# VisionDepth/VisionDepth3D

Measured on AMD Instinct MI355X. Metric: stereo-pairs/sec end-to-end (depth+warp+fill+mux), higher is better.
Workload: dtype f32; 1 GPU; 4k-dav2b-dibr; frame=3840x2160, format=Half-SBS, depth_model=depth-anything-v2-base, depth_net_dtype=float32 (the reference's precision), pixel_overlap=True, pixel_streams=2, clip_frames_all_ranks=32, params=render_cli.py defaults + dof_strength 2.0, dense DOF order (parity mode)

## Files before the change

include/vd3d.h:

```cpp
#ifndef VD3D_H
#define VD3D_H

#include <stddef.h>
#include <stdint.h>

#ifdef __cplusplus
extern "C" {
#endif

#define VD3D_ABI_VERSION 6

typedef enum vd3d_status {
  VD3D_OK = 0,
  VD3D_E_INVALID = -1,
  VD3D_E_HIP = -2,
  VD3D_E_NOMEM = -3,
  VD3D_E_UNSUPPORTED = -4
} vd3d_status;

typedef enum vd3d_format {
  VD3D_FMT_HALF_SBS = 0,
  VD3D_FMT_FULL_SBS = 1,
  VD3D_FMT_VR = 2,
  VD3D_FMT_ANAGLYPH = 3,
// ... 158 lines not shown
                         uint8_t* out_bgr, long long pitch_bytes);
int vd3d_add_weighted_u8(vd3d_ctx* ctx, const uint8_t* a, double alpha, const uint8_t* b, double beta, double gamma, long long n,
                         uint8_t* out);
int vd3d_rife_preprocess(vd3d_ctx* ctx, int dtype, const uint8_t* frame1_bgr, const uint8_t* frame2_bgr, int h, int w, int channels_last,
                         void* out6);
int vd3d_rife_postprocess(vd3d_ctx* ctx, const float* pred3, int h, int w, int channels_last, uint8_t* out_bgr);

int vd3d_conv3x3_c64_f16(vd3d_ctx* ctx, const void* x_nhwc, int H, int W, const void* w_frag, const float* bias, const float* slope_or_null,
                         void* y_nhwc);
int vd3d_conv3x3_head_f16(vd3d_ctx* ctx, const void* x_nhwc3, int H, int W, const float* w27x64, const float* bias, const float* slope_or_null,
                          void* y_nhwc64);
int vd3d_esr_tail_f32(vd3d_ctx* ctx, const void* t_nhwc64, const void* x_nhwc3, int H, int W, int r, float* out_planar);

int vd3d_depth_handoff(vd3d_ctx* ctx, const float* pred, int B, int ph, int pw, int H, int W, int invert, uint8_t* out_gray);

typedef enum vd3d_dtype { VD3D_DT_BF16 = 0, VD3D_DT_F32 = 1, VD3D_DT_F16 = 2  } vd3d_dtype;

int vd3d_depth_preprocess(vd3d_ctx* ctx, const uint8_t* frames_bgr, int B, int H, int W, int th, int tw,
                          const float* mean3_host, const float* std3_host, int dtype, void* out_nhwc);

int vd3d_add_layernorm(vd3d_ctx* ctx, int dtype, const void* x, const void* y_or_null, const void* gamma, const void* beta,
                       float eps, int64_t rows, int cols, void* out_sum, void* out_norm);

enum { VD3D_GEMM_EPI_NONE = 0, VD3D_GEMM_EPI_GELU = 1 };
enum { VD3D_X3_BF16X3 = 0, VD3D_X3_FP16X2 = 1 };
int64_t vd3d_gemm_x3_weight_bytes(int N, int K, int mode);
int vd3d_gemm_x3_pack_weights(vd3d_ctx* ctx, const float* W, int N, int K, int mode, void* image);
int vd3d_gemm_x3(vd3d_ctx* ctx, const float* X, int64_t M, int K, const void* w_image, int N, int mode, const float* bias_or_null, int epilogue, float* Y);
int64_t vd3d_attention_x3_workspace_bytes(int B, int T, int H, int D, int mode);
int vd3d_attention_x3(vd3d_ctx* ctx, const float* qkv, int B, int T, int H, int D, float scale, int mode, void* workspace, int64_t workspace_bytes, float* out);
int vd3d_attention_f32(vd3d_ctx* ctx, const float* qkv, int B, int T, int H, int D, float scale, float* out);

int64_t vd3d_conv3x3_x2_weight_bytes(int Cin, int Cout);
int vd3d_conv3x3_x2_pack_weights(vd3d_ctx* ctx, const float* W, int Cin, int Cout, void* image);
int vd3d_conv3x3_x2(vd3d_ctx* ctx, const float* X, int B, int H, int W, int Cin, const void* w_image, int Cout, float* Y);

int vd3d_upsample_bilinear_nhwc(vd3d_ctx* ctx, int dtype, const void* in, void* out, int B, int ih, int iw, int oh, int ow, int C);

int vd3d_nhwc_bias_act_f32(vd3d_ctx* ctx, const float* y, const float* bias_or_null, const float* r1_or_null, const float* r2_or_null, int relu,
                           int64_t n_pix, int C, float* out, float* relu_out_or_null);
int vd3d_upsample_bilinear_bias_nhwc_f32(vd3d_ctx* ctx, const float* in, const float* bias, float* out, int B, int ih, int iw, int oh, int ow, int C);
int vd3d_dpt_head_tail_f32(vd3d_ctx* ctx, const float* y, const float* b2, const float* w3, float b3, float scale, int64_t n_pix, int C, float* out);

int vd3d_depth_to_space_bias_nhwc_f32(vd3d_ctx* ctx, const float* y, const float* bias_or_null, int B, int H, int W, int s, int C, float* out);

typedef enum vd3d_preview {
  VD3D_PREVIEW_INTERLACED = 0,
  VD3D_PREVIEW_HSBS = 1,
  VD3D_PREVIEW_LR_DIFF = 2,
  VD3D_PREVIEW_FEATHER_BLEND = 3,
  VD3D_PREVIEW_RED_BLUE = 4
} vd3d_preview;
int vd3d_preview_image(vd3d_ctx* ctx, int type, const uint8_t* left_bgr, const uint8_t* right_bgr, int h, int w, uint8_t* out_bgr);
int vd3d_preview_heatmap(vd3d_ctx* ctx, int type, const float* shift_map, int h, int w, const uint8_t* lut_bgr_dev, uint8_t* out_bgr);
// ... 25 lines not shown
```

visiondepth3d_amd/_lib.py:

```python
from __future__ import annotations

import ctypes as C
import os

from . import _abi
from ._abi import FrameScalars, RenderParams, ShiftParams, State

_HERE = os.path.dirname(os.path.abspath(__file__))
LIB_PATH = os.environ.get("VD3D_LIB_PATH") or os.path.join(_HERE, "libvd3d_hip.so")

EXPORTS = (
    "vd3d_abi_version", "vd3d_last_error", "vd3d_shift_params_default", "vd3d_render_params_default",
    "vd3d_ctx_create", "vd3d_ctx_destroy", "vd3d_sync", "vd3d_ctx_stream", "vd3d_ctx_set_stream", "vd3d_ctx_pixel_stream", "vd3d_ctx_pixel_stream_k",
    "vd3d_state_reset", "vd3d_state_new_clip", "vd3d_state_export", "vd3d_state_import", "vd3d_state_planes",
    "vd3d_last_scalars", "vd3d_pixel_shift", "vd3d_render_frame", "vd3d_render_frame_blank", "vd3d_depth_handoff", "vd3d_heal_missing_pixels", "vd3d_preview_heatmap", "vd3d_preview_arrows", "vd3d_conv3x3_c64_f16", "vd3d_conv3x3_head_f16", "vd3d_esr_tail_f32", "vd3d_nv12_to_bgr", "vd3d_bgr_to_nv12", "vd3d_resize_cubic_u8", "vd3d_resize_area_u8", "vd3d_resize_linear_u8", "vd3d_format_3d_output", "vd3d_esr_preprocess", "vd3d_esr_postprocess", "vd3d_add_weighted_u8", "vd3d_rife_preprocess", "vd3d_rife_postprocess",
    "vd3d_shard_begin", "vd3d_shard_pixels", "vd3d_shard_pixels_blank", "vd3d_tdf_plane_export", "vd3d_tdf_plane_import", "vd3d_set_pixel_overlap", "vd3d_join_pixels", "vd3d_wait_pixels", "vd3d_finish_frame", "vd3d_quantiles",
    "vd3d_subject_depth", "vd3d_shard2_p0", "vd3d_shard2_set_crops", "vd3d_shard2_p1", "vd3d_shard2_p1_batch", "vd3d_shard2_r1", "vd3d_shard2_p3", "vd3d_shard2_p3_batch", "vd3d_shard2_r2", "vd3d_depth_preprocess", "vd3d_add_layernorm", "vd3d_gemm_x3_weight_bytes", "vd3d_gemm_x3_pack_weights", "vd3d_gemm_x3", "vd3d_attention_x3_workspace_bytes", "vd3d_attention_x3", "vd3d_attention_f32", "vd3d_conv3x3_x2_weight_bytes", "vd3d_conv3x3_x2_pack_weights", "vd3d_conv3x3_x2", "vd3d_upsample_bilinear_nhwc", "vd3d_nhwc_bias_act_f32", "vd3d_upsample_bilinear_bias_nhwc_f32", "vd3d_dpt_head_tail_f32", "vd3d_depth_to_space_bias_nhwc_f32", "vd3d_preview_image", "vd3d_detect_black_bars", "vd3d_stream_copy", "vd3d_torch_math", "vd3d_torch_math_aten", "vd3d_debug_gaussian_kernel1d", "vd3d_debug_exp_torch", "vd3d_set_profiling", "vd3d_last_stage_ms", "vd3d_stage_calls",
    "vd3d_debug_planes", "vd3d_debug_tune",
)

_lib = None


class Vd3dError(RuntimeError):
    def __init__(self, code, msg):
        super().__init__(f"libvd3d_hip error {code}: {msg}")
        self.code = code


def lib():
    global _lib
    if _lib is not None:
        return _lib
    if not os.path.exists(LIB_PATH):
        raise ImportError(f"{LIB_PATH} not built: run `python -c 'import __graft_entry__ as g; g.build()'` "
                          "(hipcc --offload-arch=gfx950). There is no CPU fallback.")
    L = C.CDLL(LIB_PATH)
    vp, i32, f32p, u8p = C.c_void_p, C.c_int, C.c_void_p, C.c_void_p
    L.vd3d_abi_version.restype = i32
    L.vd3d_last_error.restype = C.c_char_p
# ... 42 lines not shown
    L.vd3d_rife_preprocess.argtypes = [vp, i32, u8p, u8p, i32, i32, i32, vp]
    L.vd3d_rife_postprocess.argtypes = [vp, f32p, i32, i32, i32, u8p]
    L.vd3d_add_weighted_u8.argtypes = [vp, u8p, C.c_double, u8p, C.c_double, C.c_double, C.c_longlong, u8p]
    L.vd3d_finish_frame.argtypes = [vp, u8p, u8p, f32p, i32, i32, C.POINTER(RenderParams), C.c_double, i32, i32, u8p]
    L.vd3d_quantiles.argtypes = [vp, f32p, C.c_int64, C.POINTER(C.c_float), i32, C.POINTER(C.c_float)]
    L.vd3d_subject_depth.argtypes = [vp, f32p, i32, i32, C.POINTER(C.c_float)]
    L.vd3d_shard2_p0.argtypes = [vp, vp, vp, vp]
    L.vd3d_shard2_set_crops.argtypes = [vp, vp, i32]
    L.vd3d_shard2_p1.argtypes = [vp, vp, vp, i32, vp, i32, i32, vp]
    L.vd3d_shard2_p1_batch.argtypes = [vp, vp, vp, i32, vp, i32, i32, i32, vp]
    L.vd3d_shard2_p3_batch.argtypes = [vp, i32, i32, i32, vp, vp]
    L.vd3d_shard2_r1.argtypes = [vp, vp, i32]
    L.vd3d_shard2_p3.argtypes = [vp, i32, i32, vp, vp]
    L.vd3d_shard2_r2.argtypes = [vp, vp, C.POINTER(C.c_int), C.POINTER(C.c_uint8), i32, vp]
    L.vd3d_depth_preprocess.argtypes = [vp, vp, i32, i32, i32, i32, i32, C.POINTER(C.c_float), C.POINTER(C.c_float), i32, vp]
    L.vd3d_gemm_x3_weight_bytes.argtypes = [i32, i32, i32]
    L.vd3d_gemm_x3_weight_bytes.restype = C.c_int64
    L.vd3d_gemm_x3_pack_weights.argtypes = [vp, vp, i32, i32, i32, vp]
    L.vd3d_gemm_x3.argtypes = [vp, vp, C.c_int64, i32, vp, i32, i32, vp, i32, vp]
    L.vd3d_attention_x3_workspace_bytes.argtypes = [i32, i32, i32, i32, i32]
    L.vd3d_attention_x3_workspace_bytes.restype = C.c_int64
    L.vd3d_attention_x3.argtypes = [vp, vp, i32, i32, i32, i32, C.c_float, i32, vp, C.c_int64, vp]
    L.vd3d_attention_f32.argtypes = [vp, vp, i32, i32, i32, i32, C.c_float, vp]
    L.vd3d_conv3x3_x2_weight_bytes.argtypes = [i32, i32]
    L.vd3d_conv3x3_x2_weight_bytes.restype = C.c_int64
    L.vd3d_conv3x3_x2_pack_weights.argtypes = [vp, vp, i32, i32, vp]
    L.vd3d_conv3x3_x2.argtypes = [vp, vp, i32, i32, i32, i32, vp, i32, vp]
    L.vd3d_add_layernorm.argtypes = [vp, i32, vp, vp, vp, vp, C.c_float, C.c_int64, i32, vp, vp]
    L.vd3d_upsample_bilinear_nhwc.argtypes = [vp, i32, vp, vp, i32, i32, i32, i32, i32, i32]
    L.vd3d_nhwc_bias_act_f32.argtypes = [vp, vp, vp, vp, vp, i32, C.c_int64, i32, vp, vp]
    L.vd3d_upsample_bilinear_bias_nhwc_f32.argtypes = [vp, vp, vp, vp, i32, i32, i32, i32, i32, i32]
    L.vd3d_dpt_head_tail_f32.argtypes = [vp, vp, vp, vp, C.c_float, C.c_float, C.c_int64, i32, vp]
    L.vd3d_depth_to_space_bias_nhwc_f32.argtypes = [vp, vp, vp, i32, i32, i32, i32, i32, vp]
    L.vd3d_preview_image.argtypes = [vp, i32, vp, vp, i32, i32, vp]
    L.vd3d_detect_black_bars.argtypes = [vp, vp, i32, i32, C.POINTER(C.c_int), C.POINTER(C.c_int)]
    L.vd3d_stream_copy.argtypes = [vp, vp, vp, C.c_size_t]
    L.vd3d_torch_math.argtypes = [vp, i32, vp, C.c_float, vp, C.c_longlong]
    L.vd3d_torch_math_aten.argtypes = [vp, i32, vp, C.c_double, vp, C.c_longlong, i32]
    L.vd3d_debug_gaussian_kernel1d.argtypes = [i32, C.c_float, vp]
    L.vd3d_debug_exp_torch.argtypes = [vp, vp, C.c_longlong]
    L.vd3d_debug_tune.argtypes = [i32, i32]
    L.vd3d_set_profiling.argtypes = [vp, i32]
    L.vd3d_last_stage_ms.argtypes = [vp, C.c_char_p]
    L.vd3d_last_stage_ms.restype = C.c_float
    L.vd3d_stage_calls.argtypes = [vp, C.c_char_p]
    L.vd3d_stage_calls.restype = C.c_long
# ... 20 lines not shown
```

visiondepth3d_amd/csrc/vd3d_api.hip:

```cpp
#include <hip/hip_runtime.h>

#include <cmath>
#include <cstdarg>
#include <cstddef>
#include <cstdio>
#include <cstring>
#include <cstdlib>
#include <map>
#include <string>
#include <vector>

#include "vd3d_kernels.h"

#define VD3D_EXPORT extern "C" __attribute__((visibility("default")))

static thread_local char g_err[512] = "";
static int set_err(int code, const char* fmt, ...) {
  va_list ap;
  va_start(ap, fmt);
  vsnprintf(g_err, sizeof g_err, fmt, ap);
  va_end(ap);
  return code;
}
#define HIPCHK(x)                                                                                     \
// ... 1337 lines not shown
    return set_err(VD3D_E_UNSUPPORTED, "attention_f32: head size %d not built (64), an empty shape (B %d T %d H %d), B * H > 65535 or qkv / out not 16-byte aligned", D, B, T, H);
  HIPCHK(hipGetLastError());
  return 0;
}

VD3D_EXPORT int64_t vd3d_gemm_x3_weight_bytes(int N, int K, int mode) { return (int64_t)vd_gemm_x3_weight_bytes(N, K, mode); }

VD3D_EXPORT int vd3d_gemm_x3_pack_weights(vd3d_ctx* c, const float* W, int N, int K, int mode, void* image) {
  if (!c || !W || !image) return set_err(VD3D_E_INVALID, "bad argument");
  if (!vd_launch_gemm_x3_pack_w(c->stream, W, N, K, image, mode)) return set_err(VD3D_E_UNSUPPORTED, "gemm_x3: K %d must be a positive multiple of 16 (N %d), mode %d in {0, 1}", K, N, mode);
  HIPCHK(hipGetLastError());
  return 0;
}

VD3D_EXPORT int vd3d_gemm_x3(vd3d_ctx* c, const float* X, int64_t M, int K, const void* w_image, int N, int mode, const float* bias_or_null, int epilogue, float* Y) {
  if (!c || !X || !w_image || !Y || M < 1) return set_err(VD3D_E_INVALID, "bad argument");
  if (epilogue != VD3D_GEMM_EPI_NONE && epilogue != VD3D_GEMM_EPI_GELU) return set_err(VD3D_E_INVALID, "gemm_x3: unknown epilogue %d", epilogue);
  if (!vd_launch_gemm_x3(c->stream, X, (long long)M, K, w_image, N, bias_or_null, epilogue, Y, mode))
    return set_err(VD3D_E_UNSUPPORTED, "gemm_x3: K %d must be a positive multiple of 16, mode %d in {0, 1}, X and the weight image 16-byte aligned", K, mode);
  HIPCHK(hipGetLastError());
  return 0;
}

VD3D_EXPORT int vd3d_upsample_bilinear_nhwc(vd3d_ctx* c, int dtype, const void* in, void* out, int B, int ih, int iw, int oh, int ow, int C) {
  if (dtype != VD3D_DT_BF16 && dtype != VD3D_DT_F32) return set_err(VD3D_E_INVALID, "bad dtype %d", dtype);
  if (!c || !in || !out || B < 1 || ih < 1 || iw < 1) return set_err(VD3D_E_INVALID, "bad argument");
  if (!vd_launch_upsample_bilinear_nhwc(c->stream, dtype, in, out, B, ih, iw, oh, ow, C))
    return set_err(VD3D_E_UNSUPPORTED, "upsample_bilinear_nhwc: C not a multiple of 8 (bf16) / 4 (f32) or output smaller than 2x2");
  HIPCHK(hipGetLastError());
  return 0;
}

VD3D_EXPORT int vd3d_nhwc_bias_act_f32(vd3d_ctx* c, const float* y, const float* bias_or_null, const float* r1_or_null, const float* r2_or_null, int relu,
                                       int64_t n_pix, int C, float* out, float* relu_out_or_null) {
  if (!c || !y || !out || n_pix < 1 || C < 4) return set_err(VD3D_E_INVALID, "bad argument");
  HIPCHK(hipSetDevice(c->device));
  if (!vd_launch_bias_act_f32(c->stream, y, bias_or_null, r1_or_null, r2_or_null, relu, (long long)n_pix, C, out, relu_out_or_null))
    return set_err(VD3D_E_UNSUPPORTED, "nhwc_bias_act: C %d not a multiple of 4", C);
  HIPCHK(hipGetLastError());
  return 0;
}
VD3D_EXPORT int vd3d_upsample_bilinear_bias_nhwc_f32(vd3d_ctx* c, const float* in, const float* bias, float* out, int B, int ih, int iw, int oh, int ow, int C) {
  if (!c || !in || !bias || !out || B < 1 || ih < 1 || iw < 1) return set_err(VD3D_E_INVALID, "bad argument");
  HIPCHK(hipSetDevice(c->device));
  if (!vd_launch_upsample_bilinear_bias_nhwc_f32(c->stream, in, bias, out, B, ih, iw, oh, ow, C))
    return set_err(VD3D_E_UNSUPPORTED, "upsample_bilinear_bias_nhwc: C not a multiple of 4 or output smaller than 2x2");
// ... 183 lines not shown
```

visiondepth3d_amd/csrc/vd3d_gemm.hip:

```cpp
#include "vd3d_dev.h"
#include "vd3d_kernels.h"
#include <cstdlib>

typedef short gx_bf8 __attribute__((ext_vector_type(8)));
typedef float gx_f16 __attribute__((ext_vector_type(16)));

#define GX_BM 256
#define GX_BN 256
#define GX_NT 512
#define GX_MG 4
#define GX_A_STAGE (4 * GX_BM * 16)
#define GX_NTERM(MODE) ((MODE) == 0 ? 3 : 2)
#define GX_STAGE_HALF(MODE) (GX_NTERM(MODE) * 2 * GX_BN * 16)
#define GX_STAGE(MODE) (GX_A_STAGE + GX_STAGE_HALF(MODE))
#define GX_NSTAGE 4
#define GX_LDS(MODE) (GX_NSTAGE * GX_STAGE(MODE))

struct vd_gx_args {
  long long M;
  int K, N, KS;
  int nbm, nbn;
  int epilogue;
  int has_bias;
};

// ... 270 lines not shown
#endif
    attr_set = true;
  }
  vd_gx_args a;
  a.M = M; a.K = K; a.N = N; a.KS = K / 16;
  a.nbm = (int)((M + GX_BM - 1) / GX_BM); a.nbn = (N + GX_BN - 1) / GX_BN;
  a.epilogue = epilogue; a.has_bias = bias ? 1 : 0;
  const int per_xcd = (a.nbm + 7) / 8, groups = (per_xcd + GX_MG - 1) / GX_MG;
  const unsigned grid = 8u * (unsigned)groups * (unsigned)GX_MG * (unsigned)a.nbn;
  const float* cs = gx_colscale(wimg, N, K, mode);
  if (mode == 1) {
    hipLaunchKernelGGL((k_gemm_bf16x3<0, 1>), dim3(grid), dim3(GX_NT), GX_LDS(1), s, X, reinterpret_cast<const uint4*>(wimg), bias, cs, Y, a);
    return true;
  }
#ifdef VD_GEMM_ABLATE
#define GX_L(D) hipLaunchKernelGGL((k_gemm_bf16x3<D, 0>), dim3(grid), dim3(GX_NT), GX_LDS(0), s, X, reinterpret_cast<const uint4*>(wimg), bias, cs, Y, a)
  switch (dbg) { case 1: GX_L(1); return true; case 2: GX_L(2); return true; case 4: GX_L(4); return true; case 8: GX_L(8); return true; case 5: GX_L(5); return true;
                 case 3: GX_L(3); return true; case 9: GX_L(9); return true; case 11: GX_L(11); return true; case 16: GX_L(16); return true; case 27: GX_L(27); return true; case 32: GX_L(32); return true; case 64: GX_L(64); return true; case 128: GX_L(128); return true; case 130: GX_L(130); return true; case 256: GX_L(256); return true; default: break; }
#endif
  (void)dbg;
  hipLaunchKernelGGL((k_gemm_bf16x3<0, 0>), dim3(grid), dim3(GX_NT), GX_LDS(0), s, X, reinterpret_cast<const uint4*>(wimg), bias, cs, Y, a);
  return true;
}
```

visiondepth3d_amd/csrc/vd3d_kernels.h:

```cpp
#pragma once
#include <hip/hip_runtime.h>

#include "vd3d_work.h"

enum { VD_ST_A0 = 0, VD_ST_B0, VD_ST_A1, VD_ST_B1, VD_ST_A2, VD_ST_B2,
       VD_ST_AQ, VD_ST_BQ, VD_ST_BS };
#define PL_KMAX_HOST 129
#define DF_RMAX_HOST 15

#define VD_ETAB 8
struct vd_stage_args {
  int stage;
  int have_eye;
  int W, H;
  long long n_eye;
  long long n_crop;
  double ipd_factor;
  int shard;
  int shard_idx;
  float* q_out;
  long long* m_out;
  const int* crop_tab;
  const float* etab;
  int dbg;
// ... 137 lines not shown
                               int bar_width, int bar_side, uint8_t* L_out, uint8_t* R_out, const float* wtab);
#define VD_D4_WTAB_FLOATS (4 * 31 * 32)
bool vd_launch_sharp_fit(hipStream_t s, const uint8_t* gL, const uint8_t* gR, const vd3d_render_params& p, const vd_finish_consts& fc, uint8_t* out);
void vd_launch_sharp_mux(hipStream_t s, const uint8_t* gL, const uint8_t* gR, const vd3d_render_params& p,
                         const vd_finish_consts& fc, uint8_t* out, int presharp_pitch = 0, bool identity_fit = false);
void vd_launch_stream_copy(hipStream_t s, const void* src, void* dst, size_t bytes);
void vd_launch_interp_planes(hipStream_t s, const float* src, int C, int ih, int iw, float* dst, int oh, int ow, int premult);
void vd_launch_torch_math_aten(hipStream_t s, int op, const float* x, double p, float* out, long long n, int threads);
void vd_launch_torch_math(hipStream_t s, int op, const float* x, float p, float* out, long long n);
void vd_launch_blank_eye(hipStream_t s, const uint8_t* src, int h, int w, const vd_dev_work* wk, uint8_t* dst);

bool vd_launch_preview(hipStream_t s, int type, const uint8_t* L, const uint8_t* R, int h, int w, uint8_t* out);
bool vd_launch_depth_prep(hipStream_t s, const uint8_t* frames, int B, int H, int W, int th, int tw, const float mean[3],
                          const float stdv[3], int dtype, void* out_nhwc);
long long vd_gemm_x3_weight_bytes(int N, int K, int mode);
bool vd_launch_gemm_x3_pack_w(hipStream_t s, const float* W, int N, int K, void* img, int mode);
bool vd_launch_gemm_x3(hipStream_t s, const float* X, long long M, int K, const void* wimg, int N, const float* bias, int epilogue, float* Y, int mode);
long long vd_conv3x3_x2_weight_bytes(int Cin, int Cout);
bool vd_launch_conv3x3_x2_pack(hipStream_t s, const float* W, int Cin, int Cout, void* img);
bool vd_launch_conv3x3_x2(hipStream_t s, const float* X, int B, int H, int W, int Cin, const void* wimg, int Cout, float* Y);
long long vd_attn_x3_workspace_bytes(int B, int T, int H, int D, int mode);
bool vd_launch_attn_x3(hipStream_t s, const float* qkv, int B, int T, int H, int D, float scale, void* ws, float* out, int mode);
bool vd_launch_attn_f32(hipStream_t s, const float* qkv, int B, int T, int H, int D, float scale, float* out);
bool vd_launch_add_layernorm(hipStream_t s, int dtype, const void* x, const void* y, const void* gamma, const void* beta, float eps,
                             long long rows, int cols, void* out_sum, void* out_norm);
bool vd_launch_upsample_bilinear_nhwc(hipStream_t s, int dtype, const void* in, void* out, int B, int ih, int iw, int oh, int ow, int C);
bool vd_launch_bias_act_f32(hipStream_t s, const float* y, const float* bias, const float* r1, const float* r2, int relu, long long n_pix, int C,
                            float* out, float* relu_out);
bool vd_launch_upsample_bilinear_bias_nhwc_f32(hipStream_t s, const float* in, const float* bias, float* out, int B, int ih, int iw, int oh, int ow, int C);
bool vd_launch_head_tail_f32(hipStream_t s, const float* y, const float* b2, const float* w3, float b3, float scale, long long n_pix, int C, float* out);
bool vd_launch_depth_to_space_bias_f32(hipStream_t s, const float* y, const float* bias, int B, int H, int W, int f, int C, float* out);
void vd_launch_depth_handoff(hipStream_t s, const float* pred, int B, int ph, int pw, int H, int W, int invert, uint32_t* mm,
                             uint8_t* out);

bool vd_launch_finish_fused(hipStream_t s, const uint8_t* L, const uint8_t* R, const float* dn, int eh, int ew,
                            const vd3d_render_params& p, const vd_finish_consts& fc, const vd_dev_work* w, float focal,
                            int use_override, int bar_w, int bar_s, uint8_t* out, int dense, const float* w2_dev);

bool vd_launch_conv3x3_c64_f16(hipStream_t s, const void* x, int H, int W, const void* wfrag, const float* bias, const float* slope_or_null, void* y);
void vd_launch_conv3x3_head_f16(hipStream_t s, const void* x, int H, int W, const float* w27, const float* bias, const float* slope_or_null, void* y);
void vd_launch_esr_tail_f32(hipStream_t s, const void* t, const void* x, int H, int W, int r, float* out);
void vd_launch_nv12_to_bgr(hipStream_t s, const uint8_t* y, const uint8_t* uv, int h, int w, long long y_pitch, long long uv_pitch, uint8_t* out);
void vd_launch_bgr_to_nv12(hipStream_t s, const uint8_t* bgr, int h, int w, uint8_t* y, uint8_t* uv, long long y_pitch, long long uv_pitch);
bool vd_launch_preview_heatmap(hipStream_t s, int type, const float* shift, int h, int w, const uint8_t* lut_dev, uint32_t* mm, uint8_t* out);
void vd_launch_preview_arrows(hipStream_t s, const uint8_t* left, const float* shift, int h, int w, uint8_t* out);
bool vd_launch_resize_cubic_u8(hipStream_t s, const uint8_t* src, int sh, int sw, int cn, uint8_t* dst, int dh, int dw);
// ... 10 lines not shown
```

visiondepth3d_amd/depth.py:

```python
from __future__ import annotations

import json
import os
import zlib

import numpy as np
import torch
import torch.nn.functional as F

_DA_S = dict(arch="da", hidden=384, layers=12, heads=6, out_indices=[9, 10, 11, 12], neck=[48, 96, 192, 384], fusion=64, head=32)
_DA_B = dict(arch="da", hidden=768, layers=12, heads=12, out_indices=[9, 10, 11, 12], neck=[96, 192, 384, 768], fusion=128, head=32)
_DA_L = dict(arch="da", hidden=1024, layers=24, heads=16, out_indices=[21, 22, 23, 24], neck=[256, 512, 1024, 1024], fusion=256, head=32)
MODEL_ZOO = {
    "depth-anything-v2-small": _DA_S, "depth-anything-v2-base": _DA_B, "depth-anything-v2-large": _DA_L,
    "depth-anything-v1-small": _DA_S, "depth-anything-v1-base": _DA_B, "depth-anything-v1-large": _DA_L,
    "distill-any-depth-small": _DA_S, "distill-any-depth-large": _DA_L,
    "dpt-large": dict(arch="dpt", hidden=1024, layers=24, heads=16, out_indices=[5, 11, 17, 23], neck=[256, 512, 1024, 1024], fusion=256),
}
IMAGENET_MEAN = (0.485, 0.456, 0.406)
IMAGENET_STD = (0.229, 0.224, 0.225)
PROCESSORS = {
    "da": dict(size=(518, 518), keep_aspect_ratio=True, multiple=14, mean=IMAGENET_MEAN, std=IMAGENET_STD),
    "dpt": dict(size=(384, 384), keep_aspect_ratio=False, multiple=1, mean=(0.5, 0.5, 0.5), std=(0.5, 0.5, 0.5)),
}
# ... 347 lines not shown
                    x = hk["resize"](x)
                out.append(x)
            return out
        stage.forward = reassemble_fwd

        if not f32:
            return
        conv1, _, conv2, _, conv3, _ = list(head.head)
        tail_operands = _head_tail_operands(conv3)
        in_index = self.model.config.head_in_index

        def head_fwd(hidden_states):
            x = hidden_states[in_index].contiguous(memory_format=CL)
            size = (2 * x.shape[2], 2 * x.shape[3])
            h = R.upsample_bilinear_bias(conv_nb(conv1, x), size, conv1.bias)
            y = conv_nb(conv2, h)
            if self._flop_count is not None:
                self._flop_count[0] += 2.0 * y.numel() / y.shape[0]
            w3, b3 = tail_operands()
            return R.dpt_head_tail(y, conv2.bias, w3, b3, 1.0)
        head.forward = head_fwd


    @torch.no_grad()
    def _fuse_backbone_layers(self):
        layers = list(self.model.backbone.encoder.layer)
        R = self.renderer
        pad_state = {"T": None}
        bb = self.model.backbone
        if self.device.type == "cuda":
            def pad_tokens(_mod, _inp, out):
                T = out.shape[1]
                Tp = -(-T // 256) * 256
                pad_state["T"] = None
                if out.dtype == torch.bfloat16 and Tp != T and Tp <= T * 1.1:
                    pad_state["T"] = T
                    return F.pad(out, (0, 0, 0, Tp - T))
                return out
            bb.embeddings.register_forward_hook(pad_tokens)
            final_ln = bb.layernorm.forward
            bb.layernorm.forward = lambda x: final_ln(x if pad_state["T"] is None else x[:, :pad_state["T"]])
        stash = {"x": None, "h": None}
        for li, layer in enumerate(layers):
            att, out = layer.attention.attention, layer.attention.output.dense
            wqkv = torch.cat([att.query.weight, att.key.weight, att.value.weight], 0).contiguous()
            bqkv = torch.cat([att.query.bias, att.key.bias, att.value.bias], 0).contiguous()
            l1, l2 = layer.layer_scale1.lambda1.float(), layer.layer_scale2.lambda1.float()
            wo = (out.weight.float() * l1[:, None]).to(out.weight.dtype).contiguous()
            bo = (out.bias.float() * l1).to(out.bias.dtype).contiguous()
            fc1, fc2 = layer.mlp.fc1, layer.mlp.fc2
            w2 = (fc2.weight.float() * l2[:, None]).to(fc2.weight.dtype).contiguous()
            b2 = (fc2.bias.float() * l2).to(fc2.bias.dtype).contiguous()
            nh, hd, scaling = att.num_attention_heads, att.attention_head_size, att.scaling
            n1, n2, act = layer.norm1, layer.norm2, layer.mlp.activation
            nxt = layers[li + 1].norm1 if li + 1 < len(layers) else None
            x3 = None
            if self.gemm != "f32":
                x3 = self._split_block(stash, pad_state, wqkv, bqkv, wo, bo, fc1.weight, fc1.bias, w2, b2, nh, hd, scaling, n1, n2, act, nxt)

            def fwd(x, wqkv=wqkv, bqkv=bqkv, wo=wo, bo=bo, fc1=fc1, w2=w2, b2=b2, nh=nh, hd=hd, scaling=scaling, n1=n1, n2=n2,
                    act=act, nxt=nxt, x3=x3):
                if x3 is not None:
                    return x3(x)
                B, T, d = x.shape
                hip = R is not None and x.dtype in (torch.bfloat16, torch.float32) and x.is_contiguous() and d in (384, 768, 1024)
                if hip:
                    h = stash["h"] if stash["x"] is x else R.add_layernorm(x, None, n1)[1]
                    stash["x"] = stash["h"] = None
                else:
                    h = n1(x)
                qkv = F.linear(h, wqkv, bqkv)
                if R is not None and x.dtype == torch.float32 and hd == 64 and not pad_state["T"]:
                    o = R.attention_f32(qkv, nh, scaling)
                else:
                    qkv = qkv.view(B, T, 3, nh, hd)
                    Tk = pad_state["T"] or T
                    q, k, v = qkv[:, :, 0].transpose(1, 2), qkv[:, :Tk, 1].transpose(1, 2), qkv[:, :Tk, 2].transpose(1, 2)
                    o = F.scaled_dot_product_attention(q, k, v, scale=scaling).transpose(1, 2).reshape(B, T, d)
                a = F.linear(o, wo, bo)
                if not hip:
                    x = x + a
                    return x + F.linear(act(fc1(n2(x))), w2, b2)
                x, h = R.add_layernorm(x, a, n2)
                m = F.linear(act(fc1(h)), w2, b2)
                if nxt is None:
                    return x + m
                x, hn = R.add_layernorm(x, m, nxt)
                stash["x"], stash["h"] = x, hn
                return x

            layer.forward = fwd

    def _split_block(self, stash, pad_state, wqkv, bqkv, wo, bo, w1, b1, w2, b2, nh, hd, scaling, n1, n2, act, nxt):
        R, gm = self.renderer, self.gemm
        gelu_ok = isinstance(act, torch.nn.GELU) and getattr(act, "approximate", "none") == "none" or type(act).__name__ == "GELUActivation"
        x3 = dict(qkv=(R.gemm_x3_pack(wqkv, gm), wqkv.shape[0]), wo=(R.gemm_x3_pack(wo, gm), wo.shape[0]),
                  fc1=(R.gemm_x3_pack(w1, gm), w1.shape[0]), w2=(R.gemm_x3_pack(w2, gm), w2.shape[0]), gelu=bool(gelu_ok), mode=gm)

        def lin(t, key, bias, gelu=False):
            return R.linear_x3(t if t.is_contiguous() else t.contiguous(), x3[key][0], x3[key][1], bias, gelu=gelu, mode=gm)

        def fwd(x):
            B, T, d = x.shape
            if not (x.dtype == torch.float32 and x.is_contiguous() and d in (384, 768, 1024)):
                raise NotImplementedError(f"gemm={gm!r}: hidden size {d} / dtype {x.dtype} not built (float32, 384 / 768 / 1024) -- refusing to fall back silently")
            h = stash["h"] if stash["x"] is x else R.add_layernorm(x, None, n1)[1]
            stash["x"] = stash["h"] = None
            qkv = lin(h, "qkv", bqkv)
            if hd == 64 and not pad_state["T"]:
                o = R.attention_x3(qkv, nh, scaling, mode=gm)
# ... 176 lines not shown
```

visiondepth3d_amd/render_3d.py:

```python
from __future__ import annotations

import ctypes as C

import numpy as np
import torch

from . import _lib
from ._abi import DEPTH_BGR_U8, DEPTH_F32, DEPTH_GRAY_U8, DT_BF16, DT_F16, DT_F32, FORMAT_IDS, FrameScalars, RenderParams, ShiftParams, State
from .geometry import aspect_ratios
from .params import reference_aten_threads, render_kwargs_to_params, shift_params_from_kwargs

torch_device = torch.device("cuda" if torch.cuda.is_available() else "cpu")


def _ptr(t: torch.Tensor):
    return C.c_void_p(t.data_ptr())


class Renderer:

    def __init__(self, device: int | torch.device | None = None, private_stream: bool = False, auto_order: bool = True):
        if not torch.cuda.is_available():
            raise RuntimeError("visiondepth3d_amd needs a ROCm GPU (MI355X); there is no CPU path")
        L = _lib.lib()
# ... 528 lines not shown
            raise AssertionError("qkv must be contiguous float32 [B, T, 3 * H * D]")
        m = self.X3_MODES[mode]
        nb = int(self._L.vd3d_attention_x3_workspace_bytes(B, T, n_heads, D, m))
        if nb < 0:
            raise NotImplementedError(f"attention_x3: head size {D} not built")
        ws = getattr(self, "_attn_ws", None)
        if ws is None or ws.numel() < nb:
            ws = self._attn_ws = torch.empty(nb, dtype=torch.uint8, device=self.device)
        out = torch.empty((B, T, n_heads * D), dtype=torch.float32, device=self.device)
        self._enter(qkv, ws, out)
        _lib.check(self._L.vd3d_attention_x3(self._ctx, _ptr(qkv), B, T, n_heads, D, float(scale), m, _ptr(ws), ws.numel(), _ptr(out)))
        return out

    def attention_f32(self, qkv: torch.Tensor, n_heads: int, scale: float) -> torch.Tensor:
        B, T, C3 = qkv.shape
        D = C3 // (3 * n_heads)
        if qkv.dtype != torch.float32 or not qkv.is_contiguous() or D * 3 * n_heads != C3:
            raise AssertionError("qkv must be contiguous float32 [B, T, 3 * H * D]")
        if D != 64:
            raise NotImplementedError(f"attention_f32: head size {D} not built")
        out = torch.empty((B, T, n_heads * D), dtype=torch.float32, device=self.device)
        self._enter(qkv, out)
        _lib.check(self._L.vd3d_attention_f32(self._ctx, _ptr(qkv), B, T, n_heads, D, float(scale), _ptr(out)))
        return out

    def conv3x3_x2_pack(self, weight: torch.Tensor):
        w = weight.detach().to(self.device, torch.float32).contiguous()
        Cout, Cin, kh, kw = w.shape
        nb = int(self._L.vd3d_conv3x3_x2_weight_bytes(Cin, Cout)) if (kh, kw) == (3, 3) else -1
        if nb < 0:
            return None
        img = torch.empty(nb, dtype=torch.uint8, device=self.device)
        self._enter(w, img)
        _lib.check(self._L.vd3d_conv3x3_x2_pack_weights(self._ctx, _ptr(w), Cin, Cout, _ptr(img)))
        return img

    def conv3x3_x2(self, x: torch.Tensor, w_image: torch.Tensor, Cout: int) -> torch.Tensor:
        B, Cin, H, W = x.shape
        if x.dtype != torch.float32 or not x.is_contiguous(memory_format=torch.channels_last):
            raise AssertionError("conv3x3_x2: float32 channels_last input")
        out = torch.empty((B, int(Cout), H, W), dtype=torch.float32, device=x.device, memory_format=torch.channels_last)
        self._enter(x, w_image, out)
        _lib.check(self._L.vd3d_conv3x3_x2(self._ctx, _ptr(x), B, H, W, Cin, _ptr(w_image), int(Cout), _ptr(out)))
        return out

    def upsample_bilinear(self, x: torch.Tensor, size) -> torch.Tensor:
# ... 193 lines not shown
```

Before: 138.9 stereo-pairs/s.

## Add f32 MFMA GEMM with bias/GELU/residual epilogues for ViT linears

Adds a custom FP32 GEMM kernel built on MFMA 32x32x2 f32 instructions. It uses LDS multi-stage staging through global_load_lds and XCD-aware tile swizzling, and offers epilogues for bias, exact GELU and residual add. The depth backbone's proj, fc1 and fc2 linears go through this kernel, so the residual adds and the GELU are folded into the GEMM instead of running as separate elementwise passes. The add_layernorm calls then receive no second operand. The kernel replaces the hipBLASLt/rocBLAS f32 GEMM, so its speed depends on how well this hand tiling competes with the vendor library.

```diff
diff --git a/include/vd3d.h b/include/vd3d.h
--- a/include/vd3d.h
+++ b/include/vd3d.h
@@ -204,7 +204,7 @@
 int vd3d_add_layernorm(vd3d_ctx* ctx, int dtype, const void* x, const void* y_or_null, const void* gamma, const void* beta,
                        float eps, int64_t rows, int cols, void* out_sum, void* out_norm);
 
-enum { VD3D_GEMM_EPI_NONE = 0, VD3D_GEMM_EPI_GELU = 1 };
+enum { VD3D_GEMM_EPI_NONE = 0, VD3D_GEMM_EPI_GELU = 1, VD3D_GEMM_EPI_RESIDUAL = 2  };
 enum { VD3D_X3_BF16X3 = 0, VD3D_X3_FP16X2 = 1 };
 int64_t vd3d_gemm_x3_weight_bytes(int N, int K, int mode);
 int vd3d_gemm_x3_pack_weights(vd3d_ctx* ctx, const float* W, int N, int K, int mode, void* image);
@@ -212,6 +212,7 @@
 int64_t vd3d_attention_x3_workspace_bytes(int B, int T, int H, int D, int mode);
 int vd3d_attention_x3(vd3d_ctx* ctx, const float* qkv, int B, int T, int H, int D, float scale, int mode, void* workspace, int64_t workspace_bytes, float* out);
 int vd3d_attention_f32(vd3d_ctx* ctx, const float* qkv, int B, int T, int H, int D, float scale, float* out);
+int vd3d_gemm_f32(vd3d_ctx* ctx, const float* X, int64_t M, int K, const float* W, int N, const float* bias_or_null, int epilogue, const float* residual_or_null, float* Y);
 
 int64_t vd3d_conv3x3_x2_weight_bytes(int Cin, int Cout);
 int vd3d_conv3x3_x2_pack_weights(vd3d_ctx* ctx, const float* W, int Cin, int Cout, void* image);
diff --git a/visiondepth3d_amd/_lib.py b/visiondepth3d_amd/_lib.py
--- a/visiondepth3d_amd/_lib.py
+++ b/visiondepth3d_amd/_lib.py
@@ -15,7 +15,7 @@
     "vd3d_state_reset", "vd3d_state_new_clip", "vd3d_state_export", "vd3d_state_import", "vd3d_state_planes",
     "vd3d_last_scalars", "vd3d_pixel_shift", "vd3d_render_frame", "vd3d_render_frame_blank", "vd3d_depth_handoff", "vd3d_heal_missing_pixels", "vd3d_preview_heatmap", "vd3d_preview_arrows", "vd3d_conv3x3_c64_f16", "vd3d_conv3x3_head_f16", "vd3d_esr_tail_f32", "vd3d_nv12_to_bgr", "vd3d_bgr_to_nv12", "vd3d_resize_cubic_u8", "vd3d_resize_area_u8", "vd3d_resize_linear_u8", "vd3d_format_3d_output", "vd3d_esr_preprocess", "vd3d_esr_postprocess", "vd3d_add_weighted_u8", "vd3d_rife_preprocess", "vd3d_rife_postprocess",
     "vd3d_shard_begin", "vd3d_shard_pixels", "vd3d_shard_pixels_blank", "vd3d_tdf_plane_export", "vd3d_tdf_plane_import", "vd3d_set_pixel_overlap", "vd3d_join_pixels", "vd3d_wait_pixels", "vd3d_finish_frame", "vd3d_quantiles",
-    "vd3d_subject_depth", "vd3d_shard2_p0", "vd3d_shard2_set_crops", "vd3d_shard2_p1", "vd3d_shard2_p1_batch", "vd3d_shard2_r1", "vd3d_shard2_p3", "vd3d_shard2_p3_batch", "vd3d_shard2_r2", "vd3d_depth_preprocess", "vd3d_add_layernorm", "vd3d_gemm_x3_weight_bytes", "vd3d_gemm_x3_pack_weights", "vd3d_gemm_x3", "vd3d_attention_x3_workspace_bytes", "vd3d_attention_x3", "vd3d_attention_f32", "vd3d_conv3x3_x2_weight_bytes", "vd3d_conv3x3_x2_pack_weights", "vd3d_conv3x3_x2", "vd3d_upsample_bilinear_nhwc", "vd3d_nhwc_bias_act_f32", "vd3d_upsample_bilinear_bias_nhwc_f32", "vd3d_dpt_head_tail_f32", "vd3d_depth_to_space_bias_nhwc_f32", "vd3d_preview_image", "vd3d_detect_black_bars", "vd3d_stream_copy", "vd3d_torch_math", "vd3d_torch_math_aten", "vd3d_debug_gaussian_kernel1d", "vd3d_debug_exp_torch", "vd3d_set_profiling", "vd3d_last_stage_ms", "vd3d_stage_calls",
+    "vd3d_subject_depth", "vd3d_shard2_p0", "vd3d_shard2_set_crops", "vd3d_shard2_p1", "vd3d_shard2_p1_batch", "vd3d_shard2_r1", "vd3d_shard2_p3", "vd3d_shard2_p3_batch", "vd3d_shard2_r2", "vd3d_depth_preprocess", "vd3d_add_layernorm", "vd3d_gemm_x3_weight_bytes", "vd3d_gemm_x3_pack_weights", "vd3d_gemm_x3", "vd3d_attention_x3_workspace_bytes", "vd3d_attention_x3", "vd3d_attention_f32", "vd3d_gemm_f32", "vd3d_conv3x3_x2_weight_bytes", "vd3d_conv3x3_x2_pack_weights", "vd3d_conv3x3_x2", "vd3d_upsample_bilinear_nhwc", "vd3d_nhwc_bias_act_f32", "vd3d_upsample_bilinear_bias_nhwc_f32", "vd3d_dpt_head_tail_f32", "vd3d_depth_to_space_bias_nhwc_f32", "vd3d_preview_image", "vd3d_detect_black_bars", "vd3d_stream_copy", "vd3d_torch_math", "vd3d_torch_math_aten", "vd3d_debug_gaussian_kernel1d", "vd3d_debug_exp_torch", "vd3d_set_profiling", "vd3d_last_stage_ms", "vd3d_stage_calls",
     "vd3d_debug_planes", "vd3d_debug_tune",
 )
 
@@ -104,6 +104,7 @@
     L.vd3d_attention_x3_workspace_bytes.restype = C.c_int64
     L.vd3d_attention_x3.argtypes = [vp, vp, i32, i32, i32, i32, C.c_float, i32, vp, C.c_int64, vp]
     L.vd3d_attention_f32.argtypes = [vp, vp, i32, i32, i32, i32, C.c_float, vp]
+    L.vd3d_gemm_f32.argtypes = [vp, vp, C.c_int64, i32, vp, i32, vp, i32, vp, vp]
     L.vd3d_conv3x3_x2_weight_bytes.argtypes = [i32, i32]
     L.vd3d_conv3x3_x2_weight_bytes.restype = C.c_int64
     L.vd3d_conv3x3_x2_pack_weights.argtypes = [vp, vp, i32, i32, vp]
diff --git a/visiondepth3d_amd/csrc/vd3d_api.hip b/visiondepth3d_amd/csrc/vd3d_api.hip
--- a/visiondepth3d_amd/csrc/vd3d_api.hip
+++ b/visiondepth3d_amd/csrc/vd3d_api.hip
@@ -1383,6 +1383,29 @@
   return 0;
 }
 
+static bool ranges_overlap(const void* p, unsigned long long np, const void* q, unsigned long long nq) {
+  const uintptr_t a = reinterpret_cast<uintptr_t>(p), b = reinterpret_cast<uintptr_t>(q);
+  return a < b + nq && b < a + np;
+}
+
+VD3D_EXPORT int vd3d_gemm_f32(vd3d_ctx* c, const float* X, int64_t M, int K, const float* W, int N, const float* bias_or_null, int epilogue,
+                              const float* residual_or_null, float* Y) {
+  if (!c || !X || !W || !Y || M < 1 || N < 1 || K < 1) return set_err(VD3D_E_INVALID, "bad argument");
+  if (epilogue != VD3D_GEMM_EPI_NONE && epilogue != VD3D_GEMM_EPI_GELU && epilogue != VD3D_GEMM_EPI_RESIDUAL) return set_err(VD3D_E_INVALID, "gemm_f32: unknown epilogue %d", epilogue);
+  if ((epilogue == VD3D_GEMM_EPI_RESIDUAL) != (residual_or_null != nullptr)) return set_err(VD3D_E_INVALID, "gemm_f32: a residual goes with VD3D_GEMM_EPI_RESIDUAL and only with it");
+  if ((reinterpret_cast<uintptr_t>(X) & 15) || (reinterpret_cast<uintptr_t>(W) & 15) || (reinterpret_cast<uintptr_t>(Y) & 3) || (reinterpret_cast<uintptr_t>(bias_or_null) & 3) ||
+      (reinterpret_cast<uintptr_t>(residual_or_null) & 3))
+    return set_err(VD3D_E_INVALID, "gemm_f32: X and W must be 16-byte aligned, bias / residual / Y float-aligned");
+  const unsigned long long ybytes = (unsigned long long)M * (unsigned long long)N * 4ull;
+  if (ranges_overlap(Y, ybytes, X, (unsigned long long)M * (unsigned long long)K * 4ull) || (residual_or_null && ranges_overlap(Y, ybytes, residual_or_null, ybytes)))
+    return set_err(VD3D_E_INVALID, "gemm_f32: Y must not alias X or the residual");
+  HIPCHK(hipSetDevice(c->device));
+  if (!vd_launch_gemm_f32(c->stream, X, (long long)M, K, W, N, bias_or_null, epilogue, residual_or_null, Y))
+    return set_err(VD3D_E_UNSUPPORTED, "gemm_f32: K %d must be a positive multiple of 16 (M %lld, N %d)", K, (long long)M, N);
+  HIPCHK(hipGetLastError());
+  return 0;
+}
+
 VD3D_EXPORT int vd3d_upsample_bilinear_nhwc(vd3d_ctx* c, int dtype, const void* in, void* out, int B, int ih, int iw, int oh, int ow, int C) {
   if (dtype != VD3D_DT_BF16 && dtype != VD3D_DT_F32) return set_err(VD3D_E_INVALID, "bad dtype %d", dtype);
   if (!c || !in || !out || B < 1 || ih < 1 || iw < 1) return set_err(VD3D_E_INVALID, "bad argument");
diff --git a/visiondepth3d_amd/csrc/vd3d_gemm.hip b/visiondepth3d_amd/csrc/vd3d_gemm.hip
--- a/visiondepth3d_amd/csrc/vd3d_gemm.hip
+++ b/visiondepth3d_amd/csrc/vd3d_gemm.hip
@@ -1,6 +1,7 @@
 #include "vd3d_dev.h"
 #include "vd3d_kernels.h"
 #include <cstdlib>
+#include <mutex>
 
 typedef short gx_bf8 __attribute__((ext_vector_type(8)));
 typedef float gx_f16 __attribute__((ext_vector_type(16)));
@@ -317,3 +318,205 @@
   hipLaunchKernelGGL((k_gemm_bf16x3<0, 0>), dim3(grid), dim3(GX_NT), GX_LDS(0), s, X, reinterpret_cast<const uint4*>(wimg), bias, cs, Y, a);
   return true;
 }
+
+typedef float gx_f4 __attribute__((ext_vector_type(4)));
+#define GF_BM 256
+#define GF_A_STAGE (GF_BM * 64)
+#define GF_BN(WN) (128 * (WN))
+#define GF_STAGE(WN) (GF_A_STAGE + GF_BN(WN) * 64)
+#define GF_NSTAGE(WN) ((WN) == 2 ? 4 : 3)
+#define GF_LDS(WN) (GF_NSTAGE(WN) * GF_STAGE(WN))
+
+template <int WN, int EPI>
+__global__ __launch_bounds__(256 * WN, 2) void k_gemm_f32(const float* __restrict__ X, const float* __restrict__ W, const float* __restrict__ bias,
+                                                          const float* __restrict__ R, float* __restrict__ Y, vd_gx_args a) {
+  constexpr int NT = 256 * WN, BN = GF_BN(WN), STAGE = GF_STAGE(WN), NSTAGE = GF_NSTAGE(WN), NPA = GF_BM * 4 / NT, NPB = BN * 4 / NT;
+  static_assert(NPB == 2 && (NPA + NPB) * (NSTAGE - 1) == 12, "the counted waits below are written for these figures");
+  extern __shared__ __attribute__((aligned(16))) uint8_t gx_lds[];
+  int mt, nt;
+  {
+    const int b = blockIdx.x, x = b & 7, idx = b >> 3;
+    const int per = GX_MG * a.nbn, mg = idx / per, rem = idx - mg * per;
+    nt = rem / GX_MG;
+    mt = ((mg * GX_MG + (rem - nt * GX_MG)) << 3) + x;
+    if (mt >= a.nbm) return;
+  }
+  const int tid = threadIdx.x, lane = tid & 63, wave = __builtin_amdgcn_readfirstlane(tid >> 6);
+  const int wm = wave / WN, wn = wave % WN, li = lane & 31, kh = lane >> 5;
+  const long long m0 = (long long)mt * GF_BM;
+  const int n0 = nt * BN;
+
+  const float* xa[NPA];
+  const float* wa[NPB];
+#pragma unroll
+  for (int p = 0; p < NPA; ++p) {
+    const int slot = p * NT + tid, r = slot >> 2;
+    long long row = m0 + r;
+    if (row > a.M - 1) row = a.M - 1;
+    xa[p] = X + row * (long long)a.K + 4 * ((slot & 3) ^ ((r >> 2) & 3));
+  }
+#pragma unroll
+  for (int p = 0; p < NPB; ++p) {
+    const int slot = p * NT + tid, r = slot >> 2;
+    int row = n0 + r;
+    if (row > a.N - 1) row = a.N - 1;
+    wa[p] = W + (size_t)row * a.K + 4 * ((slot & 3) ^ ((r >> 2) & 3));
+  }
+  const int wave_base = (tid & ~63) * 16;
+  auto stage = [&](int ks, int buf) {
+    uint8_t* dst = gx_lds + buf * STAGE + wave_base;
+#pragma unroll
+    for (int p = 0; p < NPA; ++p) __builtin_amdgcn_global_load_lds((gx_glb_vp)(xa[p] + ks * 16), (gx_lds_vp)(dst + p * (NT * 16)), 16, 0, 0);
+#pragma unroll
+    for (int p = 0; p < NPB; ++p) __builtin_amdgcn_global_load_lds((gx_glb_vp)(wa[p] + ks * 16), (gx_lds_vp)(dst + GF_A_STAGE + p * (NT * 16)), 16, 0, 0);
+  };
+
+  gx_f16 acc[2][4];
+#pragma unroll
+  for (int mi = 0; mi < 2; ++mi)
+#pragma unroll
+    for (int nj = 0; nj < 4; ++nj)
+#pragma unroll
+      for (int r = 0; r < 16; ++r) acc[mi][nj][r] = 0.f;
+
+  const int a_row = wm * 64 + li, b_row = wn * 128 + li, sw = (li >> 2) & 3;
+  int fa_off[2], fb_off[2];
+#pragma unroll
+  for (int h = 0; h < 2; ++h) {
+    fa_off[h] = (a_row * 4 + ((2 * h + kh) ^ sw)) * 16;
+    fb_off[h] = GF_A_STAGE + (b_row * 4 + ((2 * h + kh) ^ sw)) * 16;
+  }
+  auto rd = [&](int buf, int h, gx_bf8 (&fa)[2], gx_bf8 (&fb)[4]) {
+    const uint8_t* s = gx_lds + buf * STAGE;
+#pragma unroll
+    for (int mi = 0; mi < 2; ++mi) fa[mi] = *reinterpret_cast<const gx_bf8*>(s + fa_off[h] + mi * 2048);
+#pragma unroll
+    for (int nj = 0; nj < 4; ++nj) fb[nj] = *reinterpret_cast<const gx_bf8*>(s + fb_off[h] + nj * 2048);
+  };
+  auto mm = [&](const gx_bf8 (&fa)[2], const gx_bf8 (&fb)[4], int e0, int e1) {
+    gx_f4 av[2], bv[4];
+#pragma unroll
+    for (int mi = 0; mi < 2; ++mi) av[mi] = __builtin_bit_cast(gx_f4, fa[mi]);
+#pragma unroll
+    for (int nj = 0; nj < 4; ++nj) bv[nj] = __builtin_bit_cast(gx_f4, fb[nj]);
+#pragma unroll
+    for (int e = 0; e < 4; ++e)
+      if (e >= e0 && e < e1) {
+#pragma unroll
+        for (int nj = 0; nj < 4; ++nj)
+#pragma unroll
+          for (int mi = 0; mi < 2; ++mi) acc[mi][nj] = __builtin_amdgcn_mfma_f32_32x32x2f32(av[mi][e], bv[nj][e], acc[mi][nj], 0, 0, 0);
+      }
+    __builtin_amdgcn_sched_barrier(0);
+  };
+
+#pragma unroll
+  for (int st = 0; st < NSTAGE; ++st) stage(st < a.KS ? st : a.KS - 1, st);
+  asm volatile("s_waitcnt vmcnt(12)" ::: "memory");
+  __builtin_amdgcn_s_barrier();
+  gx_bf8 f0a[2], f0b[4], f1a[2], f1b[4];
+  rd(0, 0, f0a, f0b);
+
+  int cur = 0;
+  for (int ks = 0; ks < a.KS; ++ks) {
+    const int nxt = cur + 1 == NSTAGE ? 0 : cur + 1;
+    mm(f0a, f0b, 0, 1);
+    rd(cur, 1, f1a, f1b);
+    __builtin_amdgcn_sched_barrier(0);
+    mm(f0a, f0b, 1, 4);
+    if (WN == 2) asm volatile("s_waitcnt vmcnt(8) lgkmcnt(0)" ::: "memory"); else asm volatile("s_waitcnt vmcnt(6) lgkmcnt(0)" ::: "memory");
+    __builtin_amdgcn_s_barrier();
+    stage(ks + NSTAGE < a.KS ? ks + NSTAGE : a.KS - 1, cur);
+    __builtin_amdgcn_sched_barrier(0);
+    mm(f1a, f1b, 0, 1);
+    rd(nxt, 0, f0a, f0b);
+    __builtin_amdgcn_sched_barrier(0);
+    mm(f1a, f1b, 1, 4);
+    cur = nxt;
+  }
+  asm volatile("s_waitcnt vmcnt(0) lgkmcnt(0)" ::: "memory");
+
+  const int mrem = (int)(a.M - m0 < GF_BM ? a.M - m0 : GF_BM);
+  float* __restrict__ Yt = Y + m0 * (long long)a.N;
+  const float* __restrict__ Rt = R + m0 * (long long)a.N;
+#pragma unroll
+  for (int nj = 0; nj < 4; ++nj) {
+    const int n = n0 + wn * 128 + nj * 32 + li;
+    const bool nok = n < a.N;
+    const int nc = nok ? n : a.N - 1;
+    float bv = a.has_bias ? bias[nc] : 0.f;
+    asm volatile("" : "+v"(bv));
+#pragma unroll
+    for (int mi = 0; mi < 2; ++mi) {
+      const int rb = wm * 64 + mi * 32 + 4 * kh;
+      float rv[16];
+      if (EPI == 2) {
+#pragma unroll
+        for (int r = 0; r < 16; ++r) {
+          int row = rb + (r & 3) + 8 * (r >> 2);
+          if (row > mrem - 1) row = mrem - 1;
+          rv[r] = Rt[(unsigned)(row * a.N + nc)];
+        }
+#pragma unroll
+        for (int r = 0; r < 16; ++r) asm volatile("" : "+v"(rv[r]));
+      }
+#pragma unroll
+      for (int r = 0; r < 16; ++r) {
+        const int row = rb + (r & 3) + 8 * (r >> 2);
+        float v = acc[mi][nj][r] + bv;
+        if (EPI == 1) v = gx_gelu(v);
+        if (EPI == 2) v = v + rv[r];
+        if (nok && row < mrem) Yt[(unsigned)(row * a.N + n)] = v;
+      }
+    }
+  }
+}
+
+static int gf_wn(int N) {
+#ifdef VD_GEMM_F32_WN
+  return VD_GEMM_F32_WN;
+#else
+  (void)N;
+  return 1;
+#endif
+}
+
+static bool gf_lds_optin(const void* fn, int lds, bool (&done)[64]) {
+  static std::mutex mu;
+  int dev = 0;
+  if (hipGetDevice(&dev) != hipSuccess || dev < 0 || dev >= 64) return false;
+  std::lock_guard<std::mutex> lock(mu);
+  if (!done[dev]) {
+    if (hipFuncSetAttribute(fn, hipFuncAttributeMaxDynamicSharedMemorySize, lds) != hipSuccess) return false;
+    done[dev] = true;
+  }
+  return true;
+}
+
+template <int WN>
+static bool gf_launch(hipStream_t s, const float* X, const float* W, const float* bias, const float* R, float* Y, int epilogue, vd_gx_args a) {
+  static bool attr_set[3][64] = {};
+  const void* fn[3] = {reinterpret_cast<const void*>(k_gemm_f32<WN, 0>), reinterpret_cast<const void*>(k_gemm_f32<WN, 1>), reinterpret_cast<const void*>(k_gemm_f32<WN, 2>)};
+  if (!gf_lds_optin(fn[epilogue], GF_LDS(WN), attr_set[epilogue])) return false;
+  a.nbn = (a.N + GF_BN(WN) - 1) / GF_BN(WN);
+  const int per_xcd = (a.nbm + 7) / 8, groups = (per_xcd + GX_MG - 1) / GX_MG;
+  const dim3 grid(8u * (unsigned)groups * (unsigned)GX_MG * (unsigned)a.nbn), block(256 * WN);
+  switch (epilogue) {
+    case 0: hipLaunchKernelGGL((k_gemm_f32<WN, 0>), grid, block, GF_LDS(WN), s, X, W, bias, R, Y, a); break;
+    case 1: hipLaunchKernelGGL((k_gemm_f32<WN, 1>), grid, block, GF_LDS(WN), s, X, W, bias, R, Y, a); break;
+    default: hipLaunchKernelGGL((k_gemm_f32<WN, 2>), grid, block, GF_LDS(WN), s, X, W, bias, R, Y, a); break;
+  }
+  return true;
+}
+
+bool vd_launch_gemm_f32(hipStream_t s, const float* X, long long M, int K, const float* W, int N, const float* bias, int epilogue, const float* R, float* Y) {
+  if (M < 1 || N < 1 || K < 16 || (K & 15) || epilogue < 0 || epilogue > 2 || (epilogue == 2) != (R != nullptr)) return false;
+  if (M > (1ll << 40) / K || M > (1ll << 40) / N || (M + GF_BM - 1) / GF_BM > (1 << 20) || N > (1 << 22)) return false;
+  if ((reinterpret_cast<uintptr_t>(X) & 15) || (reinterpret_cast<uintptr_t>(W) & 15)) return false;
+  if ((reinterpret_cast<uintptr_t>(Y) & 3) || (reinterpret_cast<uintptr_t>(bias) & 3) || (reinterpret_cast<uintptr_t>(R) & 3)) return false;
+  vd_gx_args a;
+  a.M = M; a.K = K; a.N = N; a.KS = K / 16;
+  a.nbm = (int)((M + GF_BM - 1) / GF_BM); a.nbn = 0;
+  a.epilogue = epilogue; a.has_bias = bias ? 1 : 0;
+  return gf_wn(N) == 2 ? gf_launch<2>(s, X, W, bias, R, Y, epilogue, a) : gf_launch<1>(s, X, W, bias, R, Y, epilogue, a);
+}
diff --git a/visiondepth3d_amd/csrc/vd3d_kernels.h b/visiondepth3d_amd/csrc/vd3d_kernels.h
--- a/visiondepth3d_amd/csrc/vd3d_kernels.h
+++ b/visiondepth3d_amd/csrc/vd3d_kernels.h
@@ -183,6 +183,7 @@
 long long vd_attn_x3_workspace_bytes(int B, int T, int H, int D, int mode);
 bool vd_launch_attn_x3(hipStream_t s, const float* qkv, int B, int T, int H, int D, float scale, void* ws, float* out, int mode);
 bool vd_launch_attn_f32(hipStream_t s, const float* qkv, int B, int T, int H, int D, float scale, float* out);
+bool vd_launch_gemm_f32(hipStream_t s, const float* X, long long M, int K, const float* W, int N, const float* bias, int epilogue, const float* R, float* Y);
 bool vd_launch_add_layernorm(hipStream_t s, int dtype, const void* x, const void* y, const void* gamma, const void* beta, float eps,
                              long long rows, int cols, void* out_sum, void* out_norm);
 bool vd_launch_upsample_bilinear_nhwc(hipStream_t s, int dtype, const void* in, void* out, int B, int ih, int iw, int oh, int ow, int C);
diff --git a/visiondepth3d_amd/depth.py b/visiondepth3d_amd/depth.py
--- a/visiondepth3d_amd/depth.py
+++ b/visiondepth3d_amd/depth.py
@@ -393,6 +393,8 @@
         head.forward = head_fwd
 
 
+    _F32_LINEARS = {384: ("proj", "fc1", "fc2"), 768: ("proj", "fc1", "fc2"), 1024: ("proj", "fc1", "fc2")}
+
     @torch.no_grad()
     def _fuse_backbone_layers(self):
         layers = list(self.model.backbone.encoder.layer)
@@ -429,8 +431,10 @@
             if self.gemm != "f32":
                 x3 = self._split_block(stash, pad_state, wqkv, bqkv, wo, bo, fc1.weight, fc1.bias, w2, b2, nh, hd, scaling, n1, n2, act, nxt)
 
+            gelu_exact = isinstance(act, torch.nn.GELU) and getattr(act, "approximate", "none") == "none" or type(act).__name__ == "GELUActivation"
+
             def fwd(x, wqkv=wqkv, bqkv=bqkv, wo=wo, bo=bo, fc1=fc1, w2=w2, b2=b2, nh=nh, hd=hd, scaling=scaling, n1=n1, n2=n2,
-                    act=act, nxt=nxt, x3=x3):
+                    act=act, nxt=nxt, x3=x3, gelu_exact=gelu_exact):
                 if x3 is not None:
                     return x3(x)
                 B, T, d = x.shape
@@ -440,7 +444,9 @@
                     stash["x"] = stash["h"] = None
                 else:
                     h = n1(x)
-                qkv = F.linear(h, wqkv, bqkv)
+                lin32 = getattr(R, "linear_f32", None) if hip and x.dtype == torch.float32 else None
+                route = self._F32_LINEARS.get(d, ()) if lin32 is not None else ()
+                qkv = lin32(h, wqkv, bqkv) if "qkv" in route else F.linear(h, wqkv, bqkv)
                 if R is not None and x.dtype == torch.float32 and hd == 64 and not pad_state["T"]:
                     o = R.attention_f32(qkv, nh, scaling)
                 else:
@@ -448,15 +454,29 @@
                     Tk = pad_state["T"] or T
                     q, k, v = qkv[:, :, 0].transpose(1, 2), qkv[:, :Tk, 1].transpose(1, 2), qkv[:, :Tk, 2].transpose(1, 2)
                     o = F.scaled_dot_product_attention(q, k, v, scale=scaling).transpose(1, 2).reshape(B, T, d)
-                a = F.linear(o, wo, bo)
-                if not hip:
-                    x = x + a
-                    return x + F.linear(act(fc1(n2(x))), w2, b2)
-                x, h = R.add_layernorm(x, a, n2)
-                m = F.linear(act(fc1(h)), w2, b2)
-                if nxt is None:
-                    return x + m
-                x, hn = R.add_layernorm(x, m, nxt)
+                if "proj" in route:
+                    x = lin32(o if o.is_contiguous() else o.contiguous(), wo, bo, residual=x)
+                    h = R.add_layernorm(x, None, n2)[1]
+                else:
+                    a = F.linear(o, wo, bo)
+                    if not hip:
+                        x = x + a
+                        return x + F.linear(act(fc1(n2(x))), w2, b2)
+                    x, h = R.add_layernorm(x, a, n2)
+                if "fc1" in route and gelu_exact:
+                    hid = lin32(h, fc1.weight, fc1.bias, gelu=True)
+                else:
+                    hid = act(fc1(h))
+                if "fc2" in route:
+                    x = lin32(hid, w2, b2, residual=x)
+                    if nxt is None:
+                        return x
+                    hn = R.add_layernorm(x, None, nxt)[1]
+                else:
+                    m = F.linear(hid, w2, b2)
+                    if nxt is None:
+                        return x + m
+                    x, hn = R.add_layernorm(x, m, nxt)
                 stash["x"], stash["h"] = x, hn
                 return x
 
diff --git a/visiondepth3d_amd/render_3d.py b/visiondepth3d_amd/render_3d.py
--- a/visiondepth3d_amd/render_3d.py
+++ b/visiondepth3d_amd/render_3d.py
@@ -574,6 +574,23 @@
         out = torch.empty((B, T, n_heads * D), dtype=torch.float32, device=self.device)
         self._enter(qkv, out)
         _lib.check(self._L.vd3d_attention_f32(self._ctx, _ptr(qkv), B, T, n_heads, D, float(scale), _ptr(out)))
+        return out
+
+    def linear_f32(self, x: torch.Tensor, weight: torch.Tensor, bias: torch.Tensor | None = None, gelu: bool = False, residual: torch.Tensor | None = None) -> torch.Tensor:
+        K = x.shape[-1]
+        N = weight.shape[0]
+        if gelu and residual is not None:
+            raise NotImplementedError("linear_f32: GELU and a residual in one call are not built")
+        if x.dtype != torch.float32 or weight.dtype != torch.float32 or not x.is_contiguous() or not weight.is_contiguous() or weight.shape[1] != K:
+            raise AssertionError("linear_f32: x [..., K] and weight [N, K] must be contiguous float32")
+        if K < 16 or K % 16:
+            raise NotImplementedError(f"linear_f32: K = {K} is not a positive multiple of 16")
+        out = torch.empty(x.shape[:-1] + (N,), dtype=torch.float32, device=x.device)
+        if residual is not None and (residual.dtype != torch.float32 or not residual.is_contiguous() or residual.shape != out.shape):
+            raise AssertionError("linear_f32: the residual must be contiguous float32 of the output's shape")
+        self._enter(x, weight, bias, residual, out)
+        _lib.check(self._L.vd3d_gemm_f32(self._ctx, _ptr(x), x.numel() // K, K, _ptr(weight), N, _ptr(bias) if bias is not None else None,
+                                         1 if gelu else (2 if residual is not None else 0), _ptr(residual) if residual is not None else None, _ptr(out)))
         return out
 
     def conv3x3_x2_pack(self, weight: torch.Tensor):
```

Result: slower. 132.0 stereo-pairs/s (-4.9%).
